# ByteDance-Seed/VeOmni

Measured on NVIDIA B200. Metric: tokens/sec (Qwen3-8B FSDP2 bf16 seq4096), higher is better.
Workload: dtype bf16

## Files before the change

include/veomni_b200.h:

```cpp
#ifndef VEOMNI_B200_H_
#define VEOMNI_B200_H_

#include <stdint.h>

#ifdef __cplusplus
extern "C" {
#endif

#define VB200_OK 0
#define VB200_EINVAL (-1)
#define VB200_ECUDA (-2)
#define VB200_ESTATE (-3)
#define VB200_ETIMEOUT (-4)

#define VB200_ABI_VERSION 1

int vb200_abi_version(void);
const char* vb200_last_error(void);
int64_t vb200_launch_count(void);
void vb200_reset_launch_count(void);

int vb200_rmsnorm_fwd(const void* x, const void* w, void* y, float* rstd, int64_t rows, int64_t cols,
                      float eps, void* stream);
int64_t vb200_rmsnorm_bwd_partials(int64_t rows, int64_t cols);
// ... 58 lines not shown

int vb200_attn_varlen_fwd(const void* q, const void* k, const void* v, void* o, float* lse,
                          const int32_t* cu_seqlens, int32_t num_seqs, int32_t max_seqlen, int32_t total,
                          int32_t q_heads, int32_t k_heads, int32_t head_dim, const int64_t* strides,
                          float scale, int32_t causal, void* stream);
int vb200_attn_varlen_fwd_tc(const void* q, const void* k, const void* v, void* o, float* lse,
                             const int32_t* cu_seqlens, int32_t num_seqs, int32_t max_seqlen, int32_t total,
                             int32_t q_heads, int32_t k_heads, int32_t head_dim, const int64_t* strides,
                             float scale, int32_t causal, void* stream);
int vb200_attn_bwd_delta(const void* o, const void* dout, float* delta, int32_t total, int32_t q_heads,
                         int32_t head_dim, int64_t o_stride_tok, int64_t o_stride_head, int64_t do_stride_tok,
                         int64_t do_stride_head, void* stream);
int vb200_attn_varlen_bwd_tc(const void* q, const void* k, const void* v, const void* dout, const float* lse,
                             const float* delta, void* dq, void* dk, void* dv, const int32_t* cu_seqlens,
                             int32_t num_seqs, int32_t max_seqlen, int32_t total, int32_t q_heads, int32_t k_heads,
                             int32_t head_dim, const int64_t* strides, float scale, int32_t causal, void* stream);
int vb200_attn_debug_trace(int64_t* out512);
int vb200_attn_varlen_bwd(const void* q, const void* k, const void* v, const void* o, const void* dout,
                          const float* lse, float* delta, void* dq, void* dk, void* dv,
                          const int32_t* cu_seqlens, int32_t num_seqs, int32_t max_seqlen, int32_t total,
                          int32_t q_heads, int32_t k_heads, int32_t head_dim, const int64_t* strides,
                          float scale, int32_t causal, void* stream);

int vb200_symm_alloc(void** ptr, int64_t bytes);
int vb200_symm_free(void* ptr);
int vb200_ipc_get_handle(const void* ptr, void* handle64);
int vb200_ipc_open_handle(const void* handle64, void** ptr);
int vb200_ipc_close_handle(void* ptr);
int64_t vb200_comm_signal_bytes(void);
int vb200_comm_create(void** comm, int32_t rank, int32_t world, void* const* peer_data,
                      void* const* peer_signal, int64_t data_bytes);
// ... 39 lines not shown
```

veomni_b200/_lib.py:

```python

from __future__ import annotations

import ctypes
import re
from ctypes import c_char_p, c_float, c_int, c_int32, c_int64, c_void_p
from pathlib import Path

import torch

PKG = Path(__file__).resolve().parent
LIB_PATH = PKG / "libveomni_b200.so"
HEADER = PKG.parent / "include" / "veomni_b200.h"


class VB200Error(RuntimeError):
    pass


_lib = None

_F = c_float
_P = c_void_p
_I32 = c_int32
_I64 = c_int64
# ... 15 lines not shown
    "vb200_multi_scale": (c_int, [_P, _P, _I32, _I32, _P, _P]),
    "vb200_add_rmsnorm_fwd": (c_int, [_P, _P, _P, _P, _P, _P, _I64, _I64, _F, _P]),
    "vb200_rmsnorm_bwd_add": (c_int, [_P, _P, _P, _P, _P, _P, _P, _P, _I64, _I64, _P]),
    "vb200_multi_adamw": (c_int, [_P, _P, _P, _P, _P, _P, _I32, _I32, _F, _F, _F, _F, _F, _F, _F, _P, _P]),
    "vb200_cross_entropy": (c_int, [_P, _I32, _I64, _I64, _I64, _P, _I64, _P, _P, _I32, _P, _I64, _F, _P, _P, _P]),
    "vb200_count_valid_labels": (c_int, [_P, _I64, _I64, _P, _P]),
    "vb200_token_logprobs": (c_int, [_P, _I32, _I64, _I64, _I64, _P, _I64, _F, _P, _P, _P, _I32, _P, _P, _I32, _I32, _F,
                                     _P, _P, _P, _P]),
    "vb200_token_logprobs_bwd": (c_int, [_P, _I32, _I64, _I64, _I64, _P, _I64, _F, _P, _P, _P, _P, _P, _I32, _P, _P,
                                         _I32, _I32, _F, _P, _I64, _P]),
    "vb200_swiglu_fwd": (c_int, [_P, _P, _P, _I64, _I64, _I64, _I64, _P]),
    "vb200_swiglu_bwd": (c_int, [_P] * 5 + [_I64] * 5 + [_P]),
    "vb200_attn_varlen_fwd": (c_int, [_P] * 6 + [_I32] * 6 + [_P, _F, _I32, _P]),
    "vb200_attn_varlen_fwd_tc": (c_int, [_P] * 6 + [_I32] * 6 + [_P, _F, _I32, _P]),
    "vb200_attn_bwd_delta": (c_int, [_P, _P, _P, _I32, _I32, _I32, _I64, _I64, _I64, _I64, _P]),
    "vb200_attn_varlen_bwd_tc": (c_int, [_P] * 10 + [_I32] * 6 + [_P, _F, _I32, _P]),
    "vb200_attn_debug_trace": (c_int, [_P]),
    "vb200_attn_varlen_bwd": (c_int, [_P] * 11 + [_I32] * 6 + [_P, _F, _I32, _P]),
    "vb200_moe_route_workspace": (_I64, [_I64, _I32]),
    "vb200_moe_route": (c_int, [_P, _I32, _I64, _I32, _P, _P, _P, _P, _P]),
    "vb200_moe_scatter": (c_int, [_P, _P, _P, _P, _P, _I64, _I32, _I64, _P]),
    "vb200_moe_gather": (c_int, [_P, _P, _P, _P, _I64, _I32, _I64, _P]),
    "vb200_moe_weight_grad": (c_int, [_P, _P, _P, _P, _I64, _I32, _I64, _P]),
    "vb200_group_gemm": (c_int, [_I32, _P, _P, _P, _P, _I32, _I64, _I32, _I32, _I32, _P]),
    "vb200_symm_alloc": (c_int, [ctypes.POINTER(_P), _I64]),
    "vb200_symm_free": (c_int, [_P]),
    "vb200_ipc_get_handle": (c_int, [_P, _P]),
    "vb200_ipc_open_handle": (c_int, [_P, ctypes.POINTER(_P)]),
    "vb200_ipc_close_handle": (c_int, [_P]),
    "vb200_comm_signal_bytes": (_I64, []),
    "vb200_comm_create": (c_int, [ctypes.POINTER(_P), _I32, _I32, ctypes.POINTER(_P), ctypes.POINTER(_P), _I64]),
# ... 58 lines not shown
```

veomni_b200/attention.py:

```python

from __future__ import annotations

import ctypes
import math
import os

import torch

from . import _lib
from ._lib import VB200Error, check, stream_ptr


PROFILE = None


def _prof(tag):
    if PROFILE is None:
        return None
    lst = PROFILE if isinstance(PROFILE, list) and tag == "fwd" else (PROFILE.get(tag) if isinstance(PROFILE, dict) else None)
    if lst is None:
        return None
    ev = torch.cuda.Event(enable_timing=True)
    ev.record()
    return lst, ev
# ... 2 lines not shown
def _prof_end(h):
    if h is not None:
        lst, ev0 = h
        ev1 = torch.cuda.Event(enable_timing=True)
        ev1.record()
        lst.append((ev0, ev1))

FWD_IMPL = os.environ.get("VB200_ATTN_FWD", "tc")
BWD_IMPL = os.environ.get("VB200_ATTN_BWD", "tc")
FWD_W8 = os.environ.get("VB200_ATTN_FWD_W8", "1") == "1"
BWD_PP = os.environ.get("VB200_ATTN_BWD_PP", "0") == "1"
BWD_DQ_N128 = os.environ.get("VB200_ATTN_BWD_DQ_N128", "1") == "1"
BWD_TRACE = False
BWD_P16 = os.environ.get("VB200_ATTN_BWD_P16", "0") == "1"
BWD_DQ_SS = False


def _strides(*tensors):
    vals = []
    for t in tensors:
        if t.stride(-1) != 1:
            raise VB200Error("attention tensors must be contiguous in head_dim")
        vals += [t.stride(0), t.stride(1)]
    return (ctypes.c_int64 * len(vals))(*vals)


def _prep(t: torch.Tensor) -> torch.Tensor:
    if t.stride(-1) != 1 or t.data_ptr() % 16 or t.stride(0) % 8 or t.stride(1) % 8:
        t = t.contiguous()
    return t
# ... 40 lines not shown
        q, k, v, o, lse, cu = ctx.saved_tensors
        max_seqlen, scale, causal = ctx.meta
        dout = _prep(dout)
        T, Hq, D = q.shape
        Hk = k.shape[1]
        dq, dk, dv = torch.empty_like(q), torch.empty_like(k), torch.empty_like(v)
        if dq.stride() != q.contiguous().stride():
            dq, dk, dv = (torch.empty(t.shape, dtype=t.dtype, device=t.device) for t in (q, k, v))
        delta = torch.empty(Hq, T, dtype=torch.float32, device=q.device)
        lib = _lib.load()
        if BWD_IMPL == "tc" and D == 128:
            with torch.cuda.device(q.device):
                check(lib.vb200_attn_bwd_delta(o.data_ptr(), dout.data_ptr(), delta.data_ptr(), T, Hq, D, o.stride(0), o.stride(1),
                                               dout.stride(0), dout.stride(1), stream_ptr()), "vb200_attn_bwd_delta")
                strides = _strides(q, k, v, dout, dq, dk, dv)
                for tag, only in (("bwd_dq", 1), ("bwd_dkdv", 2)) if isinstance(PROFILE, dict) else ((None, 0),):
                    hprof = _prof(tag) if tag else None
                    check(lib.vb200_attn_varlen_bwd_tc(q.data_ptr(), k.data_ptr(), v.data_ptr(), dout.data_ptr(), lse.data_ptr(),
                                                       delta.data_ptr(), dq.data_ptr(), dk.data_ptr(), dv.data_ptr(),
                                                       cu.data_ptr(), cu.numel() - 1, max_seqlen, T, Hq, Hk, D, strides, scale,
                                                       (1 if causal else 0) | (only << 8) | ((1 << 10) if BWD_DQ_SS else 0) | ((1 << 11) if BWD_PP else 0) | ((1 << 12) if BWD_P16 else 0) | ((1 << 13) if BWD_TRACE else 0) | ((1 << 14) if BWD_DQ_N128 else 0),
                                                       stream_ptr()),
                          "vb200_attn_varlen_bwd_tc")
                    _prof_end(hprof)
            return dq, dk, dv, None, None, None, None, None
        with torch.cuda.device(q.device):
            check(
                lib.vb200_attn_varlen_bwd(q.data_ptr(), k.data_ptr(), v.data_ptr(), o.data_ptr(), dout.data_ptr(),
                                          lse.data_ptr(), delta.data_ptr(), dq.data_ptr(), dk.data_ptr(), dv.data_ptr(),
                                          cu.data_ptr(), cu.numel() - 1, max_seqlen, T, Hq, Hk, D,
                                          _strides(q, k, v, o, dout, dq, dk, dv), scale, 1 if causal else 0,
                                          stream_ptr()),
                "vb200_attn_varlen_bwd",
            )
        return dq, dk, dv, None, None, None, None, None

# ... 50 lines not shown
```

veomni_b200/csrc/attention_tc.cu:

```cuda
#include "umma.cuh"

namespace vb {

struct AttnTcParams {
    const int* cu_seqlens;
    int Hq, Hk, total;
    int tiles, nseq;
    float scale;
    int causal;
    __nv_bfloat16* o;
    int64_t o_stride_tok, o_stride_head;
    float* lse;
};

constexpr int TC_BM = 128, TC_BN = 128, TC_D = 128;

__device__ __forceinline__ void tile_of_block(int heads, int nseq, int& order, int& head, int& seq) {
    const int per = heads * nseq;
    order = (int)blockIdx.x / per;
    const int rem = (int)blockIdx.x - order * per;
    seq = rem / heads;
    head = rem - seq * heads;
}
constexpr int TC_TILE = TC_BM * TC_D * 2;
// ... 244 lines not shown
}

struct AttnTcBwdParams {
    const int* cu_seqlens;
    int Hq, Hk, total;
    int tiles, nseq;
    float scale;
    int causal;
    const float* lse;
    const float* delta;
    __nv_bfloat16 *dq, *dk, *dv;
    int64_t dq_st, dq_sh, dk_st, dk_sh, dv_st, dv_sh;
    const __nv_bfloat16 *q, *dout;
    int64_t q_st, q_sh, do_st, do_sh;
    long long* trace;
};

constexpr int kTraceTiles = 64;
__device__ long long g_attn_trace[8 * kTraceTiles];
#define VB_TRACE(ev, j) do { if (p.trace && blockIdx.x == 0 && (j) < kTraceTiles) p.trace[(ev) * kTraceTiles + (j)] = clock64(); } while (0)

constexpr int TB_N = 64;
constexpr int TB_SMALL = TB_N * TC_D * 2;
constexpr int TB_DS = 128 * TB_N * 2;

constexpr int TB_KV_SS = 4, TB_KV_TS = 6, TB_KV_MAX = 6;
enum { Q_LOAD = 0, Q_KFULL = 1, Q_VFULL = Q_KFULL + TB_KV_MAX, Q_KEMPTY = Q_VFULL + TB_KV_MAX, Q_VEMPTY = Q_KEMPTY + TB_KV_MAX,
       Q_SPFULL = Q_VEMPTY + TB_KV_MAX, Q_SEMPTY = Q_SPFULL + 2, Q_DSFULL = Q_SEMPTY + 2, Q_DSEMPTY = Q_DSFULL + 2,
       Q_DONE = Q_DSEMPTY + 2, Q_COUNT = Q_DONE + 1 };

template <bool TS, bool PP, bool P16 = false>
// ... 436 lines not shown
                    w.w = f2_to_bf2(__uint_as_float(v[g * 8 + 6]) * p.scale, __uint_as_float(v[g * 8 + 7]) * p.scale);
                    *reinterpret_cast<uint4*>(row + c * 32 + g * 8) = w;
                }
            }
        }
        tc_fence_before();
    }
    tc_fence_before();
    __syncthreads();
    if (warp == 1) {
        tc_fence_after();
        tmem_dealloc(tmem, 512);
    }
}

constexpr int TB_QS_SS = 3, TB_QS_TS = 5, TB_QS_MAX = 5;
enum { K_LOAD = 0, K_QFULL = 1, K_QEMPTY = K_QFULL + TB_QS_MAX, K_STFULL = K_QEMPTY + TB_QS_MAX, K_STEMPTY = K_STFULL + 2,
       K_PFULL = K_STEMPTY + 2, K_PEMPTY = K_PFULL + 2, K_DONE = K_PEMPTY + 2, K_COUNT = K_DONE + 1 };


template <bool TS, bool PP, bool P16 = false>
__global__ void __launch_bounds__(P16 ? 576 : 320, 1)
attn_bwd_dkdv_tc_kernel(const __grid_constant__ CUtensorMap tmK, const __grid_constant__ CUtensorMap tmV,
                        const __grid_constant__ CUtensorMap tmQ, const __grid_constant__ CUtensorMap tmdO,
                        const AttnTcBwdParams p) {
    extern __shared__ __align__(1024) uint8_t smem[];
    uint8_t* sK = smem;
    uint8_t* sV = sK + TC_TILE;
    constexpr int TB_QS = TS ? TB_QS_TS : TB_QS_SS;
    uint8_t* sQ = sV + TC_TILE;
    uint8_t* sdO = sQ + TB_QS * TB_SMALL;
    uint8_t* sPt = sdO + TB_QS * TB_SMALL;
    uint8_t* sdSt = sPt + (TS ? 0 : 2 * TB_DS);
    uint64_t* bar = reinterpret_cast<uint64_t*>(sdSt + (TS ? 0 : 2 * TB_DS));
    uint32_t* tmem_slot = reinterpret_cast<uint32_t*>(bar + K_COUNT);
    float* sStat = reinterpret_cast<float*>(tmem_slot + 4);
    static_assert(!PP || TS, "the ping-pong variant is built on the TMEM-operand kernel");
    static_assert(!P16 || (TS && !PP), "P16 builds on the TMEM-operand kernel and replaces PP");
    const int warp = threadIdx.x >> 5, lane = threadIdx.x & 31;
    int order, hk, seq;
    tile_of_block(p.Hk, p.nseq, order, hk, seq);
    const int s0 = p.cu_seqlens[seq], L = p.cu_seqlens[seq + 1] - s0;
    const int n0 = order * TC_BM;
    if (n0 >= L) return;
    const int G = p.Hq / p.Hk;
    const int i_start = p.causal ? n0 / TB_N : 0;
    const int nq = (L + TB_N - 1) / TB_N - i_start;
    const int jobs = nq * G;

    if (threadIdx.x == 0) {
        for (int i = 0; i < K_COUNT; ++i) {
            const bool by_warps = (i >= K_STEMPTY && i < K_STEMPTY + 2) || (i >= K_PFULL && i < K_PFULL + 2);
            mbar_init(&bar[i], by_warps ? (PP ? 4 : 8) : 1);
// ... 102 lines not shown
        const int n = n0 + r;
        auto load_stat = [&](int jb) -> float {
            if (jb >= jobs || tid >= 128) return 0.f;
            const int hh = hk * G + jb / nq, qi = i_start + jb % nq;
            const int mm = qi * TB_N + (tid & 63);
            if (mm >= L) return 0.f;
            if (tid < 64) {
                const float l = p.lse[(int64_t)hh * p.total + s0 + mm];
                return (l == -INFINITY) ? 0.f : -l * kLog2eTc;
            }
            return -p.delta[(int64_t)hh * p.total + s0 + mm];
        };
        float stat_next = load_stat(P16 ? grp : (PP ? cw : 0));
        const uint32_t lane_base = tmem + ((uint32_t)(q * 32) << 16);
        const float sl2 = p.scale * kLog2eTc;
        for (int jb = P16 ? grp : (PP ? cw : 0); jb < jobs; jb += (PP || P16) ? 2 : 1) {
            const int st = jb & 1;
            const uint32_t ph = (uint32_t)(jb >> 1) & 1u;
            const int qi = i_start + jb % nq;
            float* strip = sStat + (P16 ? (grp * 2 + (int)ph) : PP ? (cw * 2 + (int)ph) : st) * 128;
            if (tid < 128) strip[tid] = stat_next;
            if (PP) asm volatile("bar.sync %0, 128;" ::"r"(1 + cw) : "memory");
            else if (P16) asm volatile("bar.sync %0, 256;" ::"r"(1 + grp) : "memory");
            else asm volatile("bar.sync 1, 256;" ::: "memory");
            stat_next = load_stat(jb + ((PP || P16) ? 2 : 1));
            const float* lse_s = strip;
            const float* dl_s = lse_s + 64;
            mbar_wait(&bar[K_STFULL + st], ph);
            tc_fence_after();
            if (!TS) mbar_wait(&bar[K_PEMPTY + st], ph ^ 1);
            const uint32_t pt_a = smem_u32(sPt + st * TB_DS), dst_a = smem_u32(sdSt + st * TB_DS);
            const bool need_mask = (qi * TB_N + TB_N > L) || (n0 + TC_BM > L) || (p.causal && n0 + TC_BM > qi * TB_N);
            if (P16) {
                const int c = cw;
// ... 76 lines not shown
                        const float2 t0 = ffma2(make_float2(__uint_as_float(sv[i + 0]), __uint_as_float(sv[i + 1])), sl2v, make_float2(l4.x, l4.y));
                        const float2 t1 = ffma2(make_float2(__uint_as_float(sv[i + 2]), __uint_as_float(sv[i + 3])), sl2v, make_float2(l4.z, l4.w));
                        const float2 e0 = make_float2(exp2f(t0.x), exp2f(t0.y)), e1 = make_float2(exp2f(t1.x), exp2f(t1.y));
                        const float2 u0 = fadd2(make_float2(__uint_as_float(dv[i + 0]), __uint_as_float(dv[i + 1])), make_float2(d4.x, d4.y));
                        const float2 u1 = fadd2(make_float2(__uint_as_float(dv[i + 2]), __uint_as_float(dv[i + 3])), make_float2(d4.z, d4.w));
                        const float2 w0 = fmul2(e0, u0), w1 = fmul2(e1, u1);
                        pk[i >> 1] = f2_to_bf2(e0.x, e0.y);
                        pk[(i >> 1) + 1] = f2_to_bf2(e1.x, e1.y);
                        dk[i >> 1] = f2_to_bf2(w0.x, w0.y);
                        dk[(i >> 1) + 1] = f2_to_bf2(w1.x, w1.y);
                    }
                }
                if (TS) {
                    tmem_st16(lane_base + st * TB_N + c * 32, pk);
                    tmem_st16(lane_base + 128 + st * TB_N + c * 32, dk);
                    tmem_wait_st();
                } else {
#pragma unroll
                    for (int g = 0; g < 4; ++g) {
                        const uint32_t a1 = swz_addr(pt_a, TC_BM, r, c * 4 + g), a2 = swz_addr(dst_a, TC_BM, r, c * 4 + g);
                        asm volatile("st.shared.v4.b32 [%0], {%1,%2,%3,%4};" ::"r"(a1), "r"(pk[g * 4]), "r"(pk[g * 4 + 1]),
                                     "r"(pk[g * 4 + 2]), "r"(pk[g * 4 + 3]) : "memory");
                        asm volatile("st.shared.v4.b32 [%0], {%1,%2,%3,%4};" ::"r"(a2), "r"(dk[g * 4]), "r"(dk[g * 4 + 1]),
                                     "r"(dk[g * 4 + 2]), "r"(dk[g * 4 + 3]) : "memory");
                    }
                }
            }
            tc_fence_before();
            if (!TS) fence_async_smem();
            __syncwarp();
// ... 63 lines not shown
    if (!attr) {
        VB_CUDA_TRY(cudaFuncSetAttribute(attn_fwd_tc_kernel<false>, cudaFuncAttributeMaxDynamicSharedMemorySize, (int)smem));
        VB_CUDA_TRY(cudaFuncSetAttribute(attn_fwd_tc_kernel<true>, cudaFuncAttributeMaxDynamicSharedMemorySize, (int)smem));
        attr = true;
    }
    p.tiles = (max_seqlen + TC_BM - 1) / TC_BM;
    p.nseq = num_seqs;
    dim3 grid(p.tiles * q_heads * num_seqs);
    if (w8) attn_fwd_tc_kernel<true><<<grid, 320, smem, (cudaStream_t)stream>>>(tmQ, tmK, tmV, p);
    else attn_fwd_tc_kernel<false><<<grid, 192, smem, (cudaStream_t)stream>>>(tmQ, tmK, tmV, p);
    vb200_count_launch(1);
    VB_HOST_CHECK_LAUNCH();
    return VB200_OK;
}

extern "C" int vb200_attn_varlen_bwd_tc(const void* q, const void* k, const void* v, const void* dout, const float* lse,
                                        const float* delta, void* dq, void* dk, void* dv, const int32_t* cu_seqlens,
                                        int32_t num_seqs, int32_t max_seqlen, int32_t total, int32_t q_heads,
                                        int32_t k_heads, int32_t head_dim, const int64_t* st, float scale, int32_t causal,
                                        void* stream) {
    const int only = (causal >> 8) & 3;
    const bool ss_operands = (causal >> 10) & 1;
    const bool pingpong = (causal >> 11) & 1;
    const bool p16 = (causal >> 12) & 1;
    const bool trace = (causal >> 13) & 1;
    const bool dq_n128 = (causal >> 14) & 1;
    causal &= 1;
    if (head_dim != 128) return vb200_set_error(VB200_EINVAL, "attn_bwd_tc: head_dim must be 128");
    if (q_heads <= 0 || k_heads <= 0 || q_heads % k_heads) return vb200_set_error(VB200_EINVAL, "attn_bwd_tc: Hq % Hk != 0");
    for (int i = 0; i < 14; ++i)
        if (st[i] & 7) return vb200_set_error(VB200_EINVAL, "attn_bwd_tc: strides must be multiples of 8 elements");
    if (total <= 0 || num_seqs <= 0 || max_seqlen <= 0) return VB200_OK;
    CUtensorMap tmQ128, tmdO128, tmK64, tmV64, tmK128, tmV128, tmQ64, tmdO64;
    int rc;
    if ((rc = make_tmap_3d(&tmQ128, q, 128, q_heads, total, st[1], st[0], 128))) return rc;
    if ((rc = make_tmap_3d(&tmdO128, dout, 128, q_heads, total, st[7], st[6], 128))) return rc;
    if ((rc = make_tmap_3d(&tmK64, k, 128, k_heads, total, st[3], st[2], 64))) return rc;
    if ((rc = make_tmap_3d(&tmV64, v, 128, k_heads, total, st[5], st[4], 64))) return rc;
    if ((rc = make_tmap_3d(&tmK128, k, 128, k_heads, total, st[3], st[2], 128))) return rc;
    if ((rc = make_tmap_3d(&tmV128, v, 128, k_heads, total, st[5], st[4], 128))) return rc;
    if ((rc = make_tmap_3d(&tmQ64, q, 128, q_heads, total, st[1], st[0], 64))) return rc;
    if ((rc = make_tmap_3d(&tmdO64, dout, 128, q_heads, total, st[7], st[6], 64))) return rc;
    AttnTcBwdParams p{};
    p.cu_seqlens = cu_seqlens; p.Hq = q_heads; p.Hk = k_heads; p.total = total; p.scale = scale; p.causal = causal;
    p.lse = lse; p.delta = delta;
    p.dq = (__nv_bfloat16*)dq; p.dq_st = st[8]; p.dq_sh = st[9];
    p.dk = (__nv_bfloat16*)dk; p.dk_st = st[10]; p.dk_sh = st[11];
    p.dv = (__nv_bfloat16*)dv; p.dv_st = st[12]; p.dv_sh = st[13];
    p.q = (const __nv_bfloat16*)q; p.q_st = st[0]; p.q_sh = st[1];
    p.dout = (const __nv_bfloat16*)dout; p.do_st = st[6]; p.do_sh = st[7];
    p.trace = nullptr;
    if (trace) {
        void* sym = nullptr;
        VB_CUDA_TRY(cudaGetSymbolAddress(&sym, g_attn_trace));
        VB_CUDA_TRY(cudaMemsetAsync(sym, 0, sizeof(long long) * 8 * kTraceTiles, (cudaStream_t)stream));
        p.trace = (long long*)sym;
    }
    const size_t smem_dq = 2 * TC_TILE + 2 * TB_KV_SS * TB_SMALL + 2 * TB_DS + Q_COUNT * 8 + 16 + 64;
    const size_t smem_dq_ts = 2 * TB_KV_TS * TB_SMALL + 2 * TB_DS + Q_COUNT * 8 + 16 + 64;
    const size_t smem_dq_n128 = (2 * N8_KV + 1) * (size_t)N8_TILE + N8_COUNT * 8 + 16 + 64;
    const size_t smem_kv = 2 * TC_TILE + 2 * TB_QS_SS * TB_SMALL + 4 * TB_DS + K_COUNT * 8 + 16 + 2 * 128 * 4 + 64;
    const size_t smem_kv_ts = 2 * TC_TILE + 2 * TB_QS_TS * TB_SMALL + K_COUNT * 8 + 16 + 4 * 128 * 4 + 64;
    static bool attr = false;
    if (!attr) {
        VB_CUDA_TRY(cudaFuncSetAttribute(attn_bwd_dq_tc_kernel<false, false>, cudaFuncAttributeMaxDynamicSharedMemorySize, (int)smem_dq));
        VB_CUDA_TRY(cudaFuncSetAttribute(attn_bwd_dq_tc_kernel<true, false>, cudaFuncAttributeMaxDynamicSharedMemorySize, (int)smem_dq_ts));
        VB_CUDA_TRY(cudaFuncSetAttribute(attn_bwd_dq_tc_kernel<true, true>, cudaFuncAttributeMaxDynamicSharedMemorySize, (int)smem_dq_ts));
        VB_CUDA_TRY(cudaFuncSetAttribute(attn_bwd_dkdv_tc_kernel<false, false>, cudaFuncAttributeMaxDynamicSharedMemorySize, (int)smem_kv));
        VB_CUDA_TRY(cudaFuncSetAttribute(attn_bwd_dkdv_tc_kernel<true, false>, cudaFuncAttributeMaxDynamicSharedMemorySize, (int)smem_kv_ts));
        VB_CUDA_TRY(cudaFuncSetAttribute(attn_bwd_dkdv_tc_kernel<true, true>, cudaFuncAttributeMaxDynamicSharedMemorySize, (int)smem_kv_ts));
        VB_CUDA_TRY(cudaFuncSetAttribute(attn_bwd_dq_tc_kernel<true, false, true>, cudaFuncAttributeMaxDynamicSharedMemorySize, (int)smem_dq_ts));
        VB_CUDA_TRY(cudaFuncSetAttribute(attn_bwd_dkdv_tc_kernel<true, false, true>, cudaFuncAttributeMaxDynamicSharedMemorySize, (int)smem_kv_ts));
        VB_CUDA_TRY(cudaFuncSetAttribute(attn_bwd_dq_n128_kernel, cudaFuncAttributeMaxDynamicSharedMemorySize, (int)smem_dq_n128));
        attr = true;
    }
    cudaStream_t s = (cudaStream_t)stream;
    p.tiles = (max_seqlen + TC_BM - 1) / TC_BM;
    p.nseq = num_seqs;
    dim3 gq(p.tiles * q_heads * num_seqs);
    if (only != 2) {
        if (dq_n128) attn_bwd_dq_n128_kernel<<<gq, 576, smem_dq_n128, s>>>(tmK128, tmV128, p);
        else if (ss_operands) attn_bwd_dq_tc_kernel<false, false><<<gq, 320, smem_dq, s>>>(tmQ128, tmdO128, tmK64, tmV64, p);
        else if (p16) attn_bwd_dq_tc_kernel<true, false, true><<<gq, 576, smem_dq_ts, s>>>(tmQ128, tmdO128, tmK64, tmV64, p);
        else if (pingpong) attn_bwd_dq_tc_kernel<true, true><<<gq, 320, smem_dq_ts, s>>>(tmQ128, tmdO128, tmK64, tmV64, p);
        else attn_bwd_dq_tc_kernel<true, false><<<gq, 320, smem_dq_ts, s>>>(tmQ128, tmdO128, tmK64, tmV64, p);
        vb200_count_launch(1);
        VB_HOST_CHECK_LAUNCH();
    }
    dim3 gk(p.tiles * k_heads * num_seqs);
    if (only != 1) {
        if (ss_operands) attn_bwd_dkdv_tc_kernel<false, false><<<gk, 320, smem_kv, s>>>(tmK128, tmV128, tmQ64, tmdO64, p);
        else if (p16) attn_bwd_dkdv_tc_kernel<true, false, true><<<gk, 576, smem_kv_ts, s>>>(tmK128, tmV128, tmQ64, tmdO64, p);
        else if (pingpong) attn_bwd_dkdv_tc_kernel<true, true><<<gk, 320, smem_kv_ts, s>>>(tmK128, tmV128, tmQ64, tmdO64, p);
        else attn_bwd_dkdv_tc_kernel<true, false><<<gk, 320, smem_kv_ts, s>>>(tmK128, tmV128, tmQ64, tmdO64, p);
        vb200_count_launch(1);
    }
    VB_HOST_CHECK_LAUNCH();
    return VB200_OK;
}

extern "C" int vb200_attn_debug_trace(int64_t* out512) {
    if (!out512) return vb200_set_error(VB200_EINVAL, "attn_debug_trace: null output");
    VB_CUDA_TRY(cudaDeviceSynchronize());
    VB_CUDA_TRY(cudaMemcpyFromSymbol(out512, g_attn_trace, sizeof(long long) * 8 * kTraceTiles));
// ... 3 lines not shown
```

veomni_b200/csrc/tma.cuh:

```cuda
#pragma once
#include <cuda.h>

#include "common.cuh"

namespace vb {

typedef CUresult (*PFN_encodeTiled)(CUtensorMap*, CUtensorMapDataType, cuuint32_t, void*, const cuuint64_t*,
                                    const cuuint64_t*, const cuuint32_t*, const cuuint32_t*, CUtensorMapInterleave,
                                    CUtensorMapSwizzle, CUtensorMapL2promotion, CUtensorMapFloatOOBfill);

inline PFN_encodeTiled get_encode_fn() {
    static PFN_encodeTiled fn = nullptr;
    if (!fn) {
        void* p = nullptr;
        cudaDriverEntryPointQueryResult q;
        if (cudaGetDriverEntryPoint("cuTensorMapEncodeTiled", &p, cudaEnableDefault, &q) != cudaSuccess ||
            q != cudaDriverEntryPointSuccess)
            return nullptr;
        fn = (PFN_encodeTiled)p;
    }
    return fn;
}

inline int make_tmap_3d(CUtensorMap* m, const void* base, uint64_t inner, uint64_t dim1, uint64_t dim2,
// ... 42 lines not shown
}

__device__ __forceinline__ void tma_load_3d(void* smem_dst, const CUtensorMap* tm, int c0, int c1, int c2,
                                            uint64_t* bar) {
    asm volatile(
        "cp.async.bulk.tensor.3d.shared::cluster.global.mbarrier::complete_tx::bytes [%0], [%1, {%3, %4, %5}], [%2];"
        ::"r"(smem_u32(smem_dst)), "l"(tm), "r"(smem_u32(bar)), "r"(c0), "r"(c1), "r"(c2)
        : "memory");
}
__device__ __forceinline__ void tma_load_2d(void* smem_dst, const CUtensorMap* tm, int c0, int c1, uint64_t* bar) {
    asm volatile(
        "cp.async.bulk.tensor.2d.shared::cluster.global.mbarrier::complete_tx::bytes [%0], [%1, {%3, %4}], [%2];"
        ::"r"(smem_u32(smem_dst)), "l"(tm), "r"(smem_u32(bar)), "r"(c0), "r"(c1)
        : "memory");
}
__device__ __forceinline__ void tma_prefetch_desc(const CUtensorMap* tm) {
    asm volatile("prefetch.tensormap [%0];" ::"l"(tm) : "memory");
}

__device__ __forceinline__ uint32_t swz_addr(uint32_t base, int rows, int r, int chunk) {
    return base + (uint32_t)(chunk >> 3) * (uint32_t)rows * 128u + (uint32_t)r * 128u +
           (uint32_t)(((chunk & 7) ^ (r & 7)) << 4);
}

__device__ __forceinline__ void ldsm_x4(uint32_t (&r)[4], uint32_t addr) {
    asm volatile("ldmatrix.sync.aligned.m8n8.x4.shared.b16 {%0,%1,%2,%3}, [%4];"
                 : "=r"(r[0]), "=r"(r[1]), "=r"(r[2]), "=r"(r[3])
                 : "r"(addr));
}
__device__ __forceinline__ void ldsm_x4_t(uint32_t (&r)[4], uint32_t addr) {
// ... 47 lines not shown
```

veomni_b200/csrc/umma.cuh:

```cuda
#pragma once
#include "tma.cuh"

namespace vb {

__device__ __forceinline__ uint64_t umma_desc(uint32_t smem_addr, uint32_t lbo_bytes, uint32_t sbo_bytes) {
    return (uint64_t)((smem_addr >> 4) & 0x3FFF) | ((uint64_t)((lbo_bytes >> 4) & 0x3FFF) << 16) |
           ((uint64_t)((sbo_bytes >> 4) & 0x3FFF) << 32) | (1ull << 46) | (2ull << 61);
}
__device__ __forceinline__ constexpr uint32_t umma_idesc(int a_mn_major, int b_mn_major, int M, int N) {
    return (1u << 4) | (1u << 7) | (1u << 10) | ((uint32_t)a_mn_major << 15) | ((uint32_t)b_mn_major << 16) |
           ((uint32_t)(N >> 3) << 17) | ((uint32_t)(M >> 4) << 24);
}
__device__ __forceinline__ bool elect_one_sync() {
    uint32_t pred;
    asm volatile("{\n\t.reg .pred P;\n\telect.sync _|P, 0xffffffff;\n\tselp.u32 %0, 1, 0, P;\n\t}" : "=r"(pred));
    return pred != 0;
}
__device__ __forceinline__ void umma_f16(uint32_t tmem_d, uint64_t adesc, uint64_t bdesc, uint32_t idesc, uint32_t accumulate) {
    asm volatile(
        "{\n\t.reg .pred p;\n\tsetp.ne.b32 p, %4, 0;\n\t"
        "tcgen05.mma.cta_group::1.kind::f16 [%0], %1, %2, %3, p;\n\t}"
        ::"r"(tmem_d), "l"(adesc), "l"(bdesc), "r"(idesc), "r"(accumulate)
        : "memory");
}
__device__ __forceinline__ void umma_f16_bo(uint32_t tmem_d, uint32_t a16, uint32_t a_off, uint32_t a_lbo, uint32_t a_sbo,
                                            uint32_t b16, uint32_t b_off, uint32_t b_lbo, uint32_t b_sbo, uint32_t idesc,
                                            uint32_t accumulate) {
    const uint32_t a_lo = a16 + ((a_off >> 4) + (((a_lbo >> 4) & 0x3FFFu) << 16));
    const uint32_t b_lo = b16 + ((b_off >> 4) + (((b_lbo >> 4) & 0x3FFFu) << 16));
    const uint32_t a_hi = ((a_sbo >> 4) & 0x3FFFu) | (1u << 14) | (2u << 29);
    const uint32_t b_hi = ((b_sbo >> 4) & 0x3FFFu) | (1u << 14) | (2u << 29);
    asm volatile(
        "{\n\t.reg .pred p;\n\t.reg .b64 da, db;\n\tsetp.ne.b32 p, %6, 0;\n\t"
        "mov.b64 da, {%1, %2};\n\tmov.b64 db, {%3, %4};\n\t"
        "tcgen05.mma.cta_group::1.kind::f16 [%0], da, db, %5, p;\n\t}"
        ::"r"(tmem_d), "r"(a_lo), "r"(a_hi), "r"(b_lo), "r"(b_hi), "r"(idesc), "r"(accumulate)
        : "memory");
}
__device__ __forceinline__ void umma_f16_ts(uint32_t tmem_d, uint32_t tmem_a, uint32_t b16, uint32_t b_off, uint32_t b_lbo,
                                            uint32_t b_sbo, uint32_t idesc, uint32_t accumulate) {
    const uint32_t b_lo = b16 + ((b_off >> 4) + (((b_lbo >> 4) & 0x3FFFu) << 16));
    const uint32_t b_hi = ((b_sbo >> 4) & 0x3FFFu) | (1u << 14) | (2u << 29);
    asm volatile(
        "{\n\t.reg .pred p;\n\t.reg .b64 db;\n\tsetp.ne.b32 p, %5, 0;\n\t"
        "mov.b64 db, {%2, %3};\n\t"
// ... 75 lines not shown
```

Before: 16030.

## Materialize dS in dK/dV backward pass and compute dQ as dS·K GEMM

The dK/dV attention backward kernel now also writes the bf16 dS tiles to a global workspace in a UMMA-ready interleaved layout. A new lightweight dQ kernel then only streams dS and K tiles through a 3-stage TMA/bulk-copy pipeline and does a single GEMM, instead of recomputing QK^T, softmax, and dP·V. Kernel order is swapped so dK/dV runs first. This trades the recompute FLOPs in the dQ pass for extra HBM traffic and a workspace of up to about 1 GB, enabled by default through an environment flag.

```diff
diff --git a/include/veomni_b200.h b/include/veomni_b200.h
--- a/include/veomni_b200.h
+++ b/include/veomni_b200.h
@@ -96,7 +96,10 @@
 int vb200_attn_varlen_bwd_tc(const void* q, const void* k, const void* v, const void* dout, const float* lse,
                              const float* delta, void* dq, void* dk, void* dv, const int32_t* cu_seqlens,
                              int32_t num_seqs, int32_t max_seqlen, int32_t total, int32_t q_heads, int32_t k_heads,
-                             int32_t head_dim, const int64_t* strides, float scale, int32_t causal, void* stream);
+                             int32_t head_dim, const int64_t* strides, float scale, int32_t causal,
+                             void* ds_workspace, int64_t ds_bytes, void* stream);
+int64_t vb200_attn_bwd_ds_workspace(int32_t num_seqs, int32_t max_seqlen, int32_t total, int32_t q_heads,
+                                    int32_t causal);
 int vb200_attn_debug_trace(int64_t* out512);
 int vb200_attn_varlen_bwd(const void* q, const void* k, const void* v, const void* o, const void* dout,
                           const float* lse, float* delta, void* dq, void* dk, void* dv,
diff --git a/veomni_b200/_lib.py b/veomni_b200/_lib.py
--- a/veomni_b200/_lib.py
+++ b/veomni_b200/_lib.py
@@ -53,7 +53,8 @@
     "vb200_attn_varlen_fwd": (c_int, [_P] * 6 + [_I32] * 6 + [_P, _F, _I32, _P]),
     "vb200_attn_varlen_fwd_tc": (c_int, [_P] * 6 + [_I32] * 6 + [_P, _F, _I32, _P]),
     "vb200_attn_bwd_delta": (c_int, [_P, _P, _P, _I32, _I32, _I32, _I64, _I64, _I64, _I64, _P]),
-    "vb200_attn_varlen_bwd_tc": (c_int, [_P] * 10 + [_I32] * 6 + [_P, _F, _I32, _P]),
+    "vb200_attn_varlen_bwd_tc": (c_int, [_P] * 10 + [_I32] * 6 + [_P, _F, _I32, _P, _I64, _P]),
+    "vb200_attn_bwd_ds_workspace": (_I64, [_I32] * 5),
     "vb200_attn_debug_trace": (c_int, [_P]),
     "vb200_attn_varlen_bwd": (c_int, [_P] * 11 + [_I32] * 6 + [_P, _F, _I32, _P]),
     "vb200_moe_route_workspace": (_I64, [_I64, _I32]),
diff --git a/veomni_b200/attention.py b/veomni_b200/attention.py
--- a/veomni_b200/attention.py
+++ b/veomni_b200/attention.py
@@ -40,6 +40,8 @@
 BWD_TRACE = False
 BWD_P16 = os.environ.get("VB200_ATTN_BWD_P16", "0") == "1"
 BWD_DQ_SS = False
+BWD_DQ_DS = os.environ.get("VB200_ATTN_BWD_DQ_DS", "1") == "1"
+BWD_DS_CAP_MB = float(os.environ.get("VB200_ATTN_BWD_DS_CAP_MB", "1024"))
 
 
 def _strides(*tensors):
@@ -110,12 +112,19 @@
                 check(lib.vb200_attn_bwd_delta(o.data_ptr(), dout.data_ptr(), delta.data_ptr(), T, Hq, D, o.stride(0), o.stride(1),
                                                dout.stride(0), dout.stride(1), stream_ptr()), "vb200_attn_bwd_delta")
                 strides = _strides(q, k, v, dout, dq, dk, dv)
-                for tag, only in (("bwd_dq", 1), ("bwd_dkdv", 2)) if isinstance(PROFILE, dict) else ((None, 0),):
+                nseq = cu.numel() - 1
+                ds, ds_bytes = None, 0
+                if BWD_DQ_DS and not (BWD_DQ_SS or BWD_PP or BWD_P16 or BWD_TRACE):
+                    ds_bytes = lib.vb200_attn_bwd_ds_workspace(nseq, max_seqlen, T, Hq, 1 if causal else 0)
+                    if 0 < ds_bytes <= BWD_DS_CAP_MB * 2**20:
+                        ds = torch.empty(ds_bytes, dtype=torch.uint8, device=q.device)
+                for tag, only in (("bwd_dkdv", 2), ("bwd_dq", 1)) if isinstance(PROFILE, dict) else ((None, 0),):
                     hprof = _prof(tag) if tag else None
                     check(lib.vb200_attn_varlen_bwd_tc(q.data_ptr(), k.data_ptr(), v.data_ptr(), dout.data_ptr(), lse.data_ptr(),
                                                        delta.data_ptr(), dq.data_ptr(), dk.data_ptr(), dv.data_ptr(),
-                                                       cu.data_ptr(), cu.numel() - 1, max_seqlen, T, Hq, Hk, D, strides, scale,
+                                                       cu.data_ptr(), nseq, max_seqlen, T, Hq, Hk, D, strides, scale,
                                                        (1 if causal else 0) | (only << 8) | ((1 << 10) if BWD_DQ_SS else 0) | ((1 << 11) if BWD_PP else 0) | ((1 << 12) if BWD_P16 else 0) | ((1 << 13) if BWD_TRACE else 0) | ((1 << 14) if BWD_DQ_N128 else 0),
+                                                       None if ds is None else ds.data_ptr(), ds_bytes if ds is not None else 0,
                                                        stream_ptr()),
                           "vb200_attn_varlen_bwd_tc")
                     _prof_end(hprof)
diff --git a/veomni_b200/csrc/attention_tc.cu b/veomni_b200/csrc/attention_tc.cu
--- a/veomni_b200/csrc/attention_tc.cu
+++ b/veomni_b200/csrc/attention_tc.cu
@@ -1,3 +1,5 @@
+#include <algorithm>
+
 #include "umma.cuh"
 
 namespace vb {
@@ -282,7 +284,25 @@
     const __nv_bfloat16 *q, *dout;
     int64_t q_st, q_sh, do_st, do_sh;
     long long* trace;
+    __nv_bfloat16* ds;
+    uint32_t ds_blocks;
 };
+
+constexpr int DS_BLOCK = 128 * 128;
+constexpr int DS_GRANULE = 128 * 8;
+__device__ __forceinline__ uint32_t ds_pairs(int L, int causal) {
+    const uint32_t t = (uint32_t)(L + 127) / 128u;
+    return causal ? t * (t + 1) / 2 : t * t;
+}
+__device__ __forceinline__ uint32_t ds_seq_base(const AttnTcBwdParams& p, int seq, int lane) {
+    uint32_t n = 0;
+    for (int s = lane; s < seq; s += 32) n += ds_pairs(p.cu_seqlens[s + 1] - p.cu_seqlens[s], p.causal);
+    return __reduce_add_sync(0xffffffffu, n) * (uint32_t)p.Hq;
+}
+__device__ __forceinline__ uint32_t ds_block(const AttnTcBwdParams& p, uint32_t base, int h, int L, int mb, int nb) {
+    return base + (uint32_t)h * ds_pairs(L, p.causal) +
+           (p.causal ? (uint32_t)mb * (mb + 1) / 2 : (uint32_t)mb * ((L + 127) / 128)) + (uint32_t)nb;
+}
 
 constexpr int kTraceTiles = 64;
 __device__ long long g_attn_trace[8 * kTraceTiles];
@@ -749,12 +769,108 @@
     }
 }
 
+constexpr int DQ_DS_STAGES = 3;
+enum { DD_FULL = 0, DD_EMPTY = DD_FULL + DQ_DS_STAGES, DD_DONE = DD_EMPTY + DQ_DS_STAGES, DD_COUNT };
+
+__global__ void __launch_bounds__(192, 1)
+attn_bwd_dq_ds_kernel(const __grid_constant__ CUtensorMap tmK, const AttnTcBwdParams p) {
+    extern __shared__ __align__(1024) uint8_t smem[];
+    uint8_t* sdS = smem;
+    uint8_t* sK = sdS + DQ_DS_STAGES * N8_TILE;
+    uint64_t* bar = reinterpret_cast<uint64_t*>(sK + DQ_DS_STAGES * N8_TILE);
+    uint32_t* tmem_slot = reinterpret_cast<uint32_t*>(bar + DD_COUNT);
+    const int warp = threadIdx.x >> 5, lane = threadIdx.x & 31;
+    int order, h, seq;
+    tile_of_block(p.Hq, p.nseq, order, h, seq);
+    const int s0 = p.cu_seqlens[seq], L = p.cu_seqlens[seq + 1] - s0;
+    const int mblk = p.tiles - 1 - order;
+    const int m0 = mblk * TC_BM;
+    if (m0 >= L) return;
+    const int hk = h / (p.Hq / p.Hk);
+    const int kv_end = p.causal ? min(L, m0 + TC_BM) : L;
+    const int n_tiles = (kv_end + N8_BN - 1) / N8_BN;
+
+    if (threadIdx.x == 0) {
+        for (int i = 0; i < DD_COUNT; ++i) mbar_init(&bar[i], 1);
+        mbar_fence_init();
+        tma_prefetch_desc(&tmK);
+    }
+    if (warp == 1) tmem_alloc(tmem_slot, 128);
+    tc_fence_before();
+    __syncthreads();
+    tc_fence_after();
+    const uint32_t tmem = *tmem_slot;
+
+    if (warp == 0) {
+        const uint32_t blk0 = ds_block(p, ds_seq_base(p, seq, lane), h, L, mblk, 0);
+        if (elect_one_sync()) {
+            for (int j = 0; j < n_tiles; ++j) {
+                const int st = j % DQ_DS_STAGES;
+                const uint32_t ph = (uint32_t)(j / DQ_DS_STAGES) & 1u;
+                const uint32_t blk = min(blk0 + (uint32_t)j, p.ds_blocks - 1u);
+                mbar_wait(&bar[DD_EMPTY + st], ph ^ 1);
+                mbar_expect_tx(&bar[DD_FULL + st], 2 * N8_TILE);
+                bulk_load(sdS + st * N8_TILE, p.ds + (int64_t)blk * DS_BLOCK, N8_TILE, &bar[DD_FULL + st]);
+                for (int hf = 0; hf < 2; ++hf)
+                    tma_load_3d(sK + st * N8_TILE + hf * N8_BN * 128, &tmK, hf * 64, hk, s0 + j * N8_BN, &bar[DD_FULL + st]);
+            }
+        }
+    } else if (warp == 1) {
+        constexpr uint32_t idesc = umma_idesc(1, 1, TC_BM, TC_D);
+        for (int j = 0; j < n_tiles; ++j) {
+            const int st = j % DQ_DS_STAGES;
+            mbar_wait(&bar[DD_FULL + st], (uint32_t)(j / DQ_DS_STAGES) & 1u);
+            tc_fence_after();
+            if (elect_one_sync()) {
+                const uint32_t ds_addr = smem_u32(sdS + st * N8_TILE), k_addr = smem_u32(sK + st * N8_TILE);
+#pragma unroll
+                for (int k = 0; k < N8_BN / 16; ++k)
+                    umma_f16_bo<0>(tmem, ds_addr >> 4, k * 256, 128, DS_GRANULE * 2, k_addr >> 4, k * 16 * 128, N8_BN * 128, 1024,
+                                   idesc, (j | k) ? 1u : 0u);
+                umma_commit(&bar[DD_EMPTY + st]);
+                if (j == n_tiles - 1) umma_commit(&bar[DD_DONE]);
+            }
+            __syncwarp();
+        }
+    } else {
+        const int r = (warp & 3) * 32 + lane;
+        const int m = m0 + r;
+        const uint32_t lane_base = tmem + ((uint32_t)((warp & 3) * 32) << 16);
+        mbar_wait(&bar[DD_DONE], 0);
+        tc_fence_after();
+        __nv_bfloat16* row = p.dq + (int64_t)(s0 + m) * p.dq_st + (int64_t)h * p.dq_sh;
+#pragma unroll 1
+        for (int c = 0; c < TC_D / 32; ++c) {
+            uint32_t v[32];
+            tmem_ld32(lane_base + c * 32, v);
+            if (m < L) {
+#pragma unroll
+                for (int g = 0; g < 4; ++g) {
+                    uint4 w;
+                    w.x = f2_to_bf2(__uint_as_float(v[g * 8 + 0]) * p.scale, __uint_as_float(v[g * 8 + 1]) * p.scale);
+                    w.y = f2_to_bf2(__uint_as_float(v[g * 8 + 2]) * p.scale, __uint_as_float(v[g * 8 + 3]) * p.scale);
+                    w.z = f2_to_bf2(__uint_as_float(v[g * 8 + 4]) * p.scale, __uint_as_float(v[g * 8 + 5]) * p.scale);
+                    w.w = f2_to_bf2(__uint_as_float(v[g * 8 + 6]) * p.scale, __uint_as_float(v[g * 8 + 7]) * p.scale);
+                    *reinterpret_cast<uint4*>(row + c * 32 + g * 8) = w;
+                }
+            }
+        }
+        tc_fence_before();
+    }
+    tc_fence_before();
+    __syncthreads();
+    if (warp == 1) {
+        tc_fence_after();
+        tmem_dealloc(tmem, 128);
+    }
+}
+
 constexpr int TB_QS_SS = 3, TB_QS_TS = 5, TB_QS_MAX = 5;
 enum { K_LOAD = 0, K_QFULL = 1, K_QEMPTY = K_QFULL + TB_QS_MAX, K_STFULL = K_QEMPTY + TB_QS_MAX, K_STEMPTY = K_STFULL + 2,
        K_PFULL = K_STEMPTY + 2, K_PEMPTY = K_PFULL + 2, K_DONE = K_PEMPTY + 2, K_COUNT = K_DONE + 1 };
 
 
-template <bool TS, bool PP, bool P16 = false>
+template <bool TS, bool PP, bool P16 = false, bool DS = false>
 __global__ void __launch_bounds__(P16 ? 576 : 320, 1)
 attn_bwd_dkdv_tc_kernel(const __grid_constant__ CUtensorMap tmK, const __grid_constant__ CUtensorMap tmV,
                         const __grid_constant__ CUtensorMap tmQ, const __grid_constant__ CUtensorMap tmdO,
@@ -772,6 +888,7 @@
     float* sStat = reinterpret_cast<float*>(tmem_slot + 4);
     static_assert(!PP || TS, "the ping-pong variant is built on the TMEM-operand kernel");
     static_assert(!P16 || (TS && !PP), "P16 builds on the TMEM-operand kernel and replaces PP");
+    static_assert(!DS || (TS && !PP && !P16), "the dS output is built into the default TMEM-operand kernel");
     const int warp = threadIdx.x >> 5, lane = threadIdx.x & 31;
     int order, hk, seq;
     tile_of_block(p.Hk, p.nseq, order, hk, seq);
@@ -904,10 +1021,16 @@
         float stat_next = load_stat(P16 ? grp : (PP ? cw : 0));
         const uint32_t lane_base = tmem + ((uint32_t)(q * 32) << 16);
         const float sl2 = p.scale * kLog2eTc;
+        const uint32_t ds_base = DS ? ds_seq_base(p, seq, lane) : 0u;
         for (int jb = P16 ? grp : (PP ? cw : 0); jb < jobs; jb += (PP || P16) ? 2 : 1) {
             const int st = jb & 1;
             const uint32_t ph = (uint32_t)(jb >> 1) & 1u;
             const int qi = i_start + jb % nq;
+            __nv_bfloat16* ds_row = nullptr;
+            if (DS) {
+                const uint32_t blk = ds_block(p, ds_base, hk * G + jb / nq, L, qi >> 1, order);
+                if (blk < p.ds_blocks) ds_row = p.ds + (int64_t)blk * DS_BLOCK + (qi & 1) * 8 * DS_GRANULE + r * 8;
+            }
             float* strip = sStat + (P16 ? (grp * 2 + (int)ph) : PP ? (cw * 2 + (int)ph) : st) * 128;
             if (tid < 128) strip[tid] = stat_next;
             if (PP) asm volatile("bar.sync %0, 128;" ::"r"(1 + cw) : "memory");
@@ -1014,6 +1137,12 @@
                 if (TS) {
                     tmem_st16(lane_base + st * TB_N + c * 32, pk);
                     tmem_st16(lane_base + 128 + st * TB_N + c * 32, dk);
+                    if (DS && ds_row) {
+#pragma unroll
+                        for (int g = 0; g < 4; ++g)
+                            __stcs(reinterpret_cast<uint4*>(ds_row + (c * 4 + g) * DS_GRANULE),
+                                   make_uint4(dk[g * 4], dk[g * 4 + 1], dk[g * 4 + 2], dk[g * 4 + 3]));
+                    }
                     tmem_wait_st();
                 } else {
 #pragma unroll
@@ -1107,11 +1236,20 @@
     return VB200_OK;
 }
 
+extern "C" int64_t vb200_attn_bwd_ds_workspace(int32_t num_seqs, int32_t max_seqlen, int32_t total, int32_t q_heads,
+                                               int32_t causal) {
+    if (num_seqs <= 0 || max_seqlen <= 0 || total <= 0 || q_heads <= 0) return 0;
+    const int64_t tmax = (max_seqlen + 127) / 128;
+    const int64_t tsum = std::min<int64_t>((int64_t)num_seqs * tmax, ((int64_t)total + 127 * (int64_t)num_seqs) / 128);
+    const int64_t blocks = (causal & 1) ? tsum * (tmax + 1) / 2 : tsum * tmax;
+    return blocks * q_heads * DS_BLOCK * 2;
+}
+
 extern "C" int vb200_attn_varlen_bwd_tc(const void* q, const void* k, const void* v, const void* dout, const float* lse,
                                         const float* delta, void* dq, void* dk, void* dv, const int32_t* cu_seqlens,
                                         int32_t num_seqs, int32_t max_seqlen, int32_t total, int32_t q_heads,
                                         int32_t k_heads, int32_t head_dim, const int64_t* st, float scale, int32_t causal,
-                                        void* stream) {
+                                        void* ds_workspace, int64_t ds_bytes, void* stream) {
     const int only = (causal >> 8) & 3;
     const bool ss_operands = (causal >> 10) & 1;
     const bool pingpong = (causal >> 11) & 1;
@@ -1119,6 +1257,12 @@
     const bool trace = (causal >> 13) & 1;
     const bool dq_n128 = (causal >> 14) & 1;
     causal &= 1;
+    const bool use_ds = ds_workspace != nullptr;
+    if (use_ds && (ss_operands || pingpong || p16 || trace))
+        return vb200_set_error(VB200_EINVAL, "attn_bwd_tc: the dS workspace needs the default dK/dV kernel");
+    if (use_ds && (((uintptr_t)ds_workspace & 15) ||
+                   ds_bytes < vb200_attn_bwd_ds_workspace(num_seqs, max_seqlen, total, q_heads, causal)))
+        return vb200_set_error(VB200_EINVAL, "attn_bwd_tc: dS workspace misaligned or below vb200_attn_bwd_ds_workspace()");
     if (head_dim != 128) return vb200_set_error(VB200_EINVAL, "attn_bwd_tc: head_dim must be 128");
     if (q_heads <= 0 || k_heads <= 0 || q_heads % k_heads) return vb200_set_error(VB200_EINVAL, "attn_bwd_tc: Hq % Hk != 0");
     for (int i = 0; i < 14; ++i)
@@ -1143,6 +1287,8 @@
     p.q = (const __nv_bfloat16*)q; p.q_st = st[0]; p.q_sh = st[1];
     p.dout = (const __nv_bfloat16*)dout; p.do_st = st[6]; p.do_sh = st[7];
     p.trace = nullptr;
+    p.ds = (__nv_bfloat16*)ds_workspace;
+    p.ds_blocks = use_ds ? (uint32_t)std::min<int64_t>(ds_bytes / (DS_BLOCK * 2), UINT32_MAX) : 0u;
     if (trace) {
         void* sym = nullptr;
         VB_CUDA_TRY(cudaGetSymbolAddress(&sym, g_attn_trace));
@@ -1154,6 +1300,7 @@
     const size_t smem_dq_n128 = (2 * N8_KV + 1) * (size_t)N8_TILE + N8_COUNT * 8 + 16 + 64;
     const size_t smem_kv = 2 * TC_TILE + 2 * TB_QS_SS * TB_SMALL + 4 * TB_DS + K_COUNT * 8 + 16 + 2 * 128 * 4 + 64;
     const size_t smem_kv_ts = 2 * TC_TILE + 2 * TB_QS_TS * TB_SMALL + K_COUNT * 8 + 16 + 4 * 128 * 4 + 64;
+    const size_t smem_dq_ds = 2 * DQ_DS_STAGES * (size_t)N8_TILE + DD_COUNT * 8 + 16 + 64;
     static bool attr = false;
     if (!attr) {
         VB_CUDA_TRY(cudaFuncSetAttribute(attn_bwd_dq_tc_kernel<false, false>, cudaFuncAttributeMaxDynamicSharedMemorySize, (int)smem_dq));
@@ -1165,12 +1312,28 @@
         VB_CUDA_TRY(cudaFuncSetAttribute(attn_bwd_dq_tc_kernel<true, false, true>, cudaFuncAttributeMaxDynamicSharedMemorySize, (int)smem_dq_ts));
         VB_CUDA_TRY(cudaFuncSetAttribute(attn_bwd_dkdv_tc_kernel<true, false, true>, cudaFuncAttributeMaxDynamicSharedMemorySize, (int)smem_kv_ts));
         VB_CUDA_TRY(cudaFuncSetAttribute(attn_bwd_dq_n128_kernel, cudaFuncAttributeMaxDynamicSharedMemorySize, (int)smem_dq_n128));
+        VB_CUDA_TRY(cudaFuncSetAttribute(attn_bwd_dkdv_tc_kernel<true, false, false, true>, cudaFuncAttributeMaxDynamicSharedMemorySize, (int)smem_kv_ts));
+        VB_CUDA_TRY(cudaFuncSetAttribute(attn_bwd_dq_ds_kernel, cudaFuncAttributeMaxDynamicSharedMemorySize, (int)smem_dq_ds));
         attr = true;
     }
     cudaStream_t s = (cudaStream_t)stream;
     p.tiles = (max_seqlen + TC_BM - 1) / TC_BM;
     p.nseq = num_seqs;
     dim3 gq(p.tiles * q_heads * num_seqs);
+    dim3 gk(p.tiles * k_heads * num_seqs);
+    if (use_ds) {
+        if (only != 1) {
+            attn_bwd_dkdv_tc_kernel<true, false, false, true><<<gk, 320, smem_kv_ts, s>>>(tmK128, tmV128, tmQ64, tmdO64, p);
+            vb200_count_launch(1);
+            VB_HOST_CHECK_LAUNCH();
+        }
+        if (only != 2) {
+            attn_bwd_dq_ds_kernel<<<gq, 192, smem_dq_ds, s>>>(tmK128, p);
+            vb200_count_launch(1);
+            VB_HOST_CHECK_LAUNCH();
+        }
+        return VB200_OK;
+    }
     if (only != 2) {
         if (dq_n128) attn_bwd_dq_n128_kernel<<<gq, 576, smem_dq_n128, s>>>(tmK128, tmV128, p);
         else if (ss_operands) attn_bwd_dq_tc_kernel<false, false><<<gq, 320, smem_dq, s>>>(tmQ128, tmdO128, tmK64, tmV64, p);
@@ -1180,7 +1343,6 @@
         vb200_count_launch(1);
         VB_HOST_CHECK_LAUNCH();
     }
-    dim3 gk(p.tiles * k_heads * num_seqs);
     if (only != 1) {
         if (ss_operands) attn_bwd_dkdv_tc_kernel<false, false><<<gk, 320, smem_kv, s>>>(tmK128, tmV128, tmQ64, tmdO64, p);
         else if (p16) attn_bwd_dkdv_tc_kernel<true, false, true><<<gk, 576, smem_kv_ts, s>>>(tmK128, tmV128, tmQ64, tmdO64, p);
diff --git a/veomni_b200/csrc/tma.cuh b/veomni_b200/csrc/tma.cuh
--- a/veomni_b200/csrc/tma.cuh
+++ b/veomni_b200/csrc/tma.cuh
@@ -80,6 +80,11 @@
         ::"r"(smem_u32(smem_dst)), "l"(tm), "r"(smem_u32(bar)), "r"(c0), "r"(c1)
         : "memory");
 }
+__device__ __forceinline__ void bulk_load(void* smem_dst, const void* src, uint32_t bytes, uint64_t* bar) {
+    asm volatile("cp.async.bulk.shared::cluster.global.mbarrier::complete_tx::bytes [%0], [%1], %2, [%3];"
+                 ::"r"(smem_u32(smem_dst)), "l"(src), "r"(bytes), "r"(smem_u32(bar))
+                 : "memory");
+}
 __device__ __forceinline__ void tma_prefetch_desc(const CUtensorMap* tm) {
     asm volatile("prefetch.tensormap [%0];" ::"l"(tm) : "memory");
 }
diff --git a/veomni_b200/csrc/umma.cuh b/veomni_b200/csrc/umma.cuh
--- a/veomni_b200/csrc/umma.cuh
+++ b/veomni_b200/csrc/umma.cuh
@@ -23,12 +23,13 @@
         ::"r"(tmem_d), "l"(adesc), "l"(bdesc), "r"(idesc), "r"(accumulate)
         : "memory");
 }
+template <uint32_t A_LAYOUT = 2>
 __device__ __forceinline__ void umma_f16_bo(uint32_t tmem_d, uint32_t a16, uint32_t a_off, uint32_t a_lbo, uint32_t a_sbo,
                                             uint32_t b16, uint32_t b_off, uint32_t b_lbo, uint32_t b_sbo, uint32_t idesc,
                                             uint32_t accumulate) {
     const uint32_t a_lo = a16 + ((a_off >> 4) + (((a_lbo >> 4) & 0x3FFFu) << 16));
     const uint32_t b_lo = b16 + ((b_off >> 4) + (((b_lbo >> 4) & 0x3FFFu) << 16));
-    const uint32_t a_hi = ((a_sbo >> 4) & 0x3FFFu) | (1u << 14) | (2u << 29);
+    const uint32_t a_hi = ((a_sbo >> 4) & 0x3FFFu) | (1u << 14) | (A_LAYOUT << 29);
     const uint32_t b_hi = ((b_sbo >> 4) & 0x3FFFu) | (1u << 14) | (2u << 29);
     asm volatile(
         "{\n\t.reg .pred p;\n\t.reg .b64 da, db;\n\tsetp.ne.b32 p, %6, 0;\n\t"
```

Result: no change. 16140 (median of 6 runs) (+0.7%).
